# hsinnan75/Dart

Hardware: AMD Instinct MI355X
Metric: M paired-end reads/sec (2x101 bp vs GRCh38-sized index), host to host; records bit-identical to CPU dart (higher is better)
Workload: dtype u64/u8 integer

## Files before the change

### dart_amd/csrc/dg_api.hip

```cpp
#include "../../include/dartgpu.h"
#include "dg_common.h"
#include "dg_fm.h"
#include "dg_seedq.h"
#include "dg_chain.h"
#include "dg_report.h"
#include "dg_pair.h"
#include "dg_reseed.h"
#include "dg_sort.h"
#include "dg_samfmt.h"
#include "dg_bamfmt.h"
#include "dg_bgzf.h"
#include "dg_fastq.h"
#include "dg_sjtab.h"
#include <stdio.h>
#include <stdlib.h>
#include <string.h>
#include <string>
#include <algorithm>
#include <vector>
#include <atomic>
#include <mutex>
#include <chrono>
#include <thread>
#include <condition_variable>
// ... 52 lines not shown
       TOP_ORDER_INFO = 28 , TOP_CLASS_HIST = 32 , TOP_CLASS_FILL = 64  };

struct IndexShared {
    std::mutex mu;
    std::condition_variable cv;
    DIndex ix{};
    std::atomic<uint32_t> gen{1};
    std::thread aids;
    std::atomic<int> aids_state{0};
    char aids_msg[256] = "";
    bool upload_done = false, upload_ok = false;
    void *d_ktab = nullptr, *d_sa_dense = nullptr;
    std::string report, report_out;
    int device = 0;
    uint32_t *d_chr_name_off = nullptr; char *d_chr_names = nullptr; bool chr_names_set = false; uint64_t chr_names_gen = 0; uint32_t chr_name_max = 0;
};

struct dg_ctx {
    int device = 0;
    IndexShared *shared_ix = nullptr; uint32_t ix_gen = 0;
    bool owns_index = true;
    hipStream_t stream = nullptr;
    hipEvent_t ev_dl = nullptr, ev_dl_block = nullptr;
    bool dl_on_copy_stream = false;
    int env_copy_stream = 1;
    hipEvent_t ev_wait = nullptr;
    char err[512] = "";
    DIndex ix{};
    DParams pr{};
    void *d_bwt = nullptr, *d_sa = nullptr, *d_pac = nullptr, *d_lockey = nullptr, *d_locchr = nullptr, *d_chroff = nullptr;
    int n_reads = 0, max_rlen = 0;
    size_t seq_bytes = 0;
    bool enc_ready = false;
    DBuf<unsigned char> seq; DBuf<uint32_t> seq_off; DBuf<uint16_t> rlen; DBuf<uint32_t> enc; DBuf<uint32_t> packed_in, nlist_in;
    DBuf<DHit> hits; DBuf<uint32_t> nhits, nseeds, seed_off, ncand, rep_off, tile_sums, tile_read, slow_units;
    DBuf<SKey> seeds; DBuf<DSeed> work; DBuf<DCand> cands; DBuf<DJob> jobs; DBuf<unsigned long long> job_items, job_pool; DBuf<RsChunkOut> job_outs; DBuf<uint32_t> job_pool_next; DBuf<unsigned long long> items; DBuf<uint32_t> hist, heavy; DBuf<DHeavy> seed_heavy; DBuf<int32_t> seed_heavy_sfail; DBuf<int16_t> chain_picks; DBuf<uint8_t> chain_todo;
    DBuf<dg_read_out> reads_out; DBuf<dg_report_out> reports; DBuf<uint32_t> cigpool, cigfinal;
    DBuf<dg_sj_out> sjpool, sjfinal;
    DBuf<dg_read_c> reads_c; DBuf<dg_report_c> reports_c; DBuf<uint32_t> cig_c;
    DBuf<unsigned char> ws;
    DBuf<unsigned long long> scan_state, scan_trace;
    int wall_khz = 100000;
    uint32_t scan_epoch = 0;
    size_t cap_seeds = 0, cap_rep = 0, cap_work = 0, cap_cig = 0;
    struct SharedCaps { std::atomic<size_t> seeds{0}, rep{0}, work{0}, cig{0}; } *shared_caps = nullptr;
    bool owns_shared_caps = false;
    unsigned long long *d_ctr = nullptr; unsigned int *d_tops = nullptr; int *d_err = nullptr; DSizes *d_sizes = nullptr; unsigned int *d_input_bad = nullptr;
    struct HostTail { DSizes sizes; int err; unsigned int input_bad; unsigned int tops[N_TOPS]; unsigned long long ctr[CTR_STRIDE]; __host__ __device__ uint32_t *sizes_words() { return (uint32_t *)&sizes; } } *h_tail = nullptr;
    bool state_zeroed = false;
    size_t used[3] = {0, 0, 0};
    bool enqueued = false;
    hipEvent_t ev[N_TIMERS + 1]; const char *tname[N_TIMERS]; int n_t = 0; float tms[N_TIMERS];
    uint64_t counters[CTR_N];
    uint64_t reruns_capacity = 0, reruns_scan = 0;
    bool want_compact = true, packed_valid = false;
    DBuf<uint32_t> sam_hdr_off, sam_qual_off, sam_qlen; DBuf<char> sam_hdr, sam_qual, sam_text; DBuf<uint64_t> sam_read_off, sam_tile;
    unsigned long long *d_sam_stat = nullptr, *h_sam_stat = nullptr;
    hipEvent_t ev_sam[2] = {nullptr, nullptr};
    bool batch_done = false, sam_valid = false; size_t sam_bytes = 0;
    DBuf<unsigned char> fq_text; DBuf<uint32_t> fq_lines, fq_tile_cnt, fq_name_at, fq_name_len, fq_loc, fq_hdr_off, fq_qual_off; DBuf<unsigned long long> fq_tile_sum; DBuf<char> fq_hdr, fq_qual;
    FqInfo *d_fq_info = nullptr, *h_fq_info = nullptr;
    hipEvent_t ev_fq[2] = {nullptr, nullptr};
    bool fq_valid = false; size_t fq_hdr_bytes = 0, fq_qual_bytes = 0; float fq_ms = 0.f;
    DBuf<unsigned char> bam_rec, bgzf_in, bgzf_slots, bgzf_out; DBuf<uint32_t> bgzf_size; DBuf<uint64_t> bgzf_off;
    unsigned long long *d_bam_stat = nullptr, *h_bam_stat = nullptr;
    hipEvent_t ev_bam[2] = {nullptr, nullptr}; float bam_ms[2] = {0.f, 0.f};
    bool bam_valid = false; size_t bam_bytes = 0; unsigned char *bam_ptr = nullptr;
    SjSlot *sj_tab = nullptr; size_t sj_slots = 0, sj_distinct = 0;
    DBuf<dg_sj_entry> sj_ovf[2], sj_in, sj_entries; int sj_ovf_cur = 0;
    DBuf<uint64_t> sj_keys[2], sj_line_off, sj_tile; DBuf<int64_t> sj_vals[2]; DBuf<uint32_t> sj_hist, sj_sums; DBuf<char> sj_text;
    unsigned long long *d_sj_stat = nullptr, *h_sj_stat = nullptr;
    hipEvent_t ev_sj[3] = {nullptr, nullptr, nullptr};
    bool sj_batch_counted = false, sj_fin_valid = false; size_t sj_fin_entries = 0, sj_fin_bytes = 0;
    size_t env_bam_first_cap = 0;
    size_t env_sam_first_cap = 0;
    bool want_full = true, full_valid = false;
    int n_cu = 256, runs_of_last_batch = 0, attempt_no = 0;
    int env_seed_waves = 4, env_bail_trips = 0 , env_report_bpc = 8, env_no_fast = 0, env_seed_legacy = 0, env_seed_slots_lg = 0, env_seed_wgs = 0, env_blocking_sync = 0;
    int env_seed_phases = 0, env_seed_wg_waves = 4, env_seed_partial = 32, env_seed_multi = 4;
    bool seed_qf_used = false;
    int env_scan_mask = 7;
    int env_chain_bpc = 8, env_seedh_bpc = 8, env_reseed_pct = 100;
    int env_rs_chunk = RS_CHUNK_DIAGS, env_rs_inline = RS_ENT_INLINE, env_rs_pool = 0;
    int env_scan_budget = 0;
};

static void read_env(dg_ctx *c)
{
    auto geti = [](const char *k, int dflt) { const char *v = getenv(k); return v ? atoi(v) : dflt; };
    c->env_seed_waves = geti("DG_SEED_WAVES", 4); c->env_bail_trips = geti("DG_SEED_BAIL_TRIPS", 0);
    c->env_seed_legacy = geti("DG_SEED_LEGACY", 0); c->env_seed_slots_lg = geti("DG_SEED_SLOTS_LG", 0); c->env_seed_wgs = geti("DG_SEED_WGS", 0); c->env_blocking_sync = geti("DG_BLOCKING_SYNC", 0);
    c->env_report_bpc = geti("DG_REPORT_BPC", 8); c->env_no_fast = geti("DG_NO_FAST_PAIR", 0);
    c->env_scan_budget = geti("DG_SCAN_POLL_BUDGET", 0); c->env_scan_mask = geti("DG_SCAN_POLL_SCANS", 7);
    c->env_seed_phases = geti("DG_SEED_PHASES", 0); c->env_seed_wg_waves = geti("DG_SEED_WG_WAVES", 4); c->env_seed_partial = geti("DG_SEED_PARTIAL_MIN", 32);
    c->env_copy_stream = geti("DG_COPY_STREAM", 1);
    c->env_chain_bpc = std::max(1, geti("DG_CHAIN_BPC", 8)); c->env_seedh_bpc = std::max(1, geti("DG_SEEDH_BPC", 8)); c->env_reseed_pct = std::max(10, geti("DG_RESEED_PCT", 100));
    c->env_rs_chunk = geti("DG_RS_CHUNK", RS_CHUNK_DIAGS); c->env_rs_chunk = std::min(1 << 24, std::max(RS_SUPER, c->env_rs_chunk / RS_SUPER * RS_SUPER));
    c->env_rs_inline = std::min(RS_ENT_INLINE, std::max(0, geti("DG_RS_ENT_MAX", RS_ENT_INLINE))); c->env_rs_pool = std::max(0, geti("DG_RS_POOL_BLOCKS", 0));
    c->env_sam_first_cap = (size_t)std::max(0, geti("DG_SAM_TEXT_FIRST_CAP", 0));
    c->env_bam_first_cap = (size_t)std::max(0, geti("DG_BAM_FIRST_CAP", 0));
    c->env_seed_multi = geti("DG_SEED_MULTI", 4); if (c->env_seed_multi < 0 || c->env_seed_multi > SQF_MULTI_MAX) c->env_seed_multi = SQF_MULTI_MAX;
}

static inline void refresh_index(dg_ctx *c)
{
    IndexShared *sh = c->shared_ix;
    if (sh && c->ix_gen != sh->gen.load(std::memory_order_acquire)) { std::lock_guard<std::mutex> lk(sh->mu); c->ix = sh->ix; c->ix_gen = sh->gen.load(); }
}

static int fail(dg_ctx *c, int code, const char *what, hipError_t e)
{
    snprintf(c ? c->err : g_init_error, 512, "%s: %s", what, e == hipSuccess ? "error" : hipGetErrorString(e));
    return code;
}
#define HIPCHK(call) do { hipError_t _e = (call); if (_e != hipSuccess) return fail(c, DG_ERR_HIP, #call, _e); } while (0)

#define SCAN_TILE 2048
__global__ void __launch_bounds__(256) k_scan_tiles(const uint32_t *in, uint32_t *out, uint32_t *tile_sums, uint32_t n)
{
    __shared__ uint32_t sh[256];
    const uint32_t base = blockIdx.x * SCAN_TILE + threadIdx.x * 8;
    uint32_t v[8], sum = 0;
    for (int i = 0; i < 8; i++) { v[i] = base + i < n ? in[base + i] : 0; sum += v[i]; }
    sh[threadIdx.x] = sum;
    __syncthreads();
    for (int o = 1; o < 256; o <<= 1) {
        uint32_t t = threadIdx.x >= o ? sh[threadIdx.x - o] : 0;
        __syncthreads();
        sh[threadIdx.x] += t;
        __syncthreads();
    }
    uint32_t run = sh[threadIdx.x] - sum;
    for (int i = 0; i < 8; i++) { if (base + i < n) out[base + i] = run; run += v[i]; }
    if (threadIdx.x == 255) tile_sums[blockIdx.x] = sh[255];
}
__global__ void __launch_bounds__(256) k_scan_top(uint32_t *tile_sums, uint32_t n_tiles, uint32_t *total_out, uint32_t *total_copy, uint32_t cap, int *err, int code)
{
    __shared__ uint32_t sh[256];
    __shared__ uint32_t carry;
    if (threadIdx.x == 0) carry = 0;
    __syncthreads();
    for (uint32_t b = 0; b < n_tiles; b += 256) {
        const uint32_t i = b + threadIdx.x;
        const uint32_t v = i < n_tiles ? tile_sums[i] : 0;
        sh[threadIdx.x] = v;
        __syncthreads();
        for (int o = 1; o < 256; o <<= 1) {
            uint32_t t = threadIdx.x >= o ? sh[threadIdx.x - o] : 0;
            __syncthreads();
            sh[threadIdx.x] += t;
            __syncthreads();
        }
        if (i < n_tiles) tile_sums[i] = carry + sh[threadIdx.x] - v;
        __syncthreads();
        if (threadIdx.x == 255) carry += sh[255];
        __syncthreads();
    }
    if (threadIdx.x == 0) {
        *total_out = carry;
        if (total_copy) *total_copy = carry;
        if (err && carry > cap) atomicMax(err, code);
    }
}
__global__ void __launch_bounds__(256) k_scan_add(uint32_t *out, const uint32_t *tile_sums, uint32_t n)
{
    const uint32_t i = blockIdx.x * 256 + threadIdx.x;
    if (i < n) out[i] += tile_sums[i / SCAN_TILE];
}

#define SO_PER 8
__global__ void __launch_bounds__(256)
k_seed_offsets(int n_reads, int paired, const uint32_t *__restrict__ nseeds, uint32_t *__restrict__ seed_off, uint32_t *__restrict__ tile_read, uint32_t n_tile_read,
               uint32_t *__restrict__ heavy_list, unsigned int *n_heavy, uint32_t *total_copy, uint32_t cap, TileScan ts, int *err)
{
    __shared__ unsigned long long s_scan[20];
// ... 631 lines not shown
{
    auto bad = [&](int code, const char *fmt, const char *arg) -> dg_ctx * {
        snprintf(g_init_error, sizeof g_init_error, fmt, arg);
        if (status) *status = code;
        return nullptr;
    };
    if (!f || !p || !f->bwt_path || !f->sa_path || !f->pac_path || f->n_chr <= 0 || !f->chr_off || !f->chr_len || f->l_pac <= 0) return bad(DG_ERR_ARG, "dg_init_files arguments: %s", "invalid");
    struct Fd { int fd = -1; ~Fd() { if (fd >= 0) close(fd); } } fb, fs, fp;
    struct stat st;
    IndexMeta m;
    if ((fb.fd = open(f->bwt_path, O_RDONLY)) < 0 || fstat(fb.fd, &st) != 0 || st.st_size < 40) return bad(DG_ERR_ARG, "cannot read %s", f->bwt_path);
    uint64_t hdr[7];
    if (pread(fb.fd, hdr, 40, 0) != 40) return bad(DG_ERR_ARG, "cannot read %s", f->bwt_path);
    m.primary = hdr[0]; m.L2[0] = 0; for (int i = 1; i < 5; i++) m.L2[i] = hdr[i]; m.seq_len = m.L2[4];
    m.bwt_words = ((uint64_t)st.st_size - 40) / 4;
    if ((fs.fd = open(f->sa_path, O_RDONLY)) < 0 || fstat(fs.fd, &st) != 0 || st.st_size < 56) return bad(DG_ERR_ARG, "cannot read %s", f->sa_path);
    if (pread(fs.fd, hdr, 56, 0) != 56) return bad(DG_ERR_ARG, "cannot read %s", f->sa_path);
    m.sa_intv = (int)hdr[5];
    if (m.sa_intv <= 0 || m.seq_len == 0) return bad(DG_ERR_ARG, "%s: bad header", f->sa_path);
    m.n_sa = (m.seq_len + (uint64_t)m.sa_intv) / (uint64_t)m.sa_intv;
    const uint64_t sa_count = std::min<uint64_t>(m.n_sa - 1, ((uint64_t)st.st_size - 56) / 8);
    if ((fp.fd = open(f->pac_path, O_RDONLY)) < 0 || fstat(fp.fd, &st) != 0) return bad(DG_ERR_ARG, "cannot read %s", f->pac_path);
    const size_t pac_copy = std::min<size_t>((size_t)st.st_size, (size_t)(f->l_pac / 4 + 1));
    m.l_pac = f->l_pac; m.n_chr = f->n_chr; m.chr_off = f->chr_off; m.chr_len = f->chr_len; m.expected_reads = f->expected_reads;
    UpSrc b, s, q;
    b.fd = fb.fd; s.fd = fs.fd; q.fd = fp.fd;
    return init_index(m, b, 40, s, 56, 1, sa_count, q, pac_copy, p, device, flags, status);
}

extern "C" dg_ctx *dg_clone(dg_ctx *parent, int *status)
{
    if (status) *status = DG_ERR_ARG;
    if (!parent) return nullptr;
    hipError_t e;
    if ((e = hipSetDevice(parent->device)) != hipSuccess) { if (status) *status = DG_ERR_HIP; return nullptr; }
    dg_ctx *c = new dg_ctx();
    c->device = parent->device; c->owns_index = false; c->n_cu = parent->n_cu;
    c->shared_ix = parent->shared_ix;
    c->ix = parent->ix; c->ix_gen = parent->ix_gen; c->pr = parent->pr;
    refresh_index(c);
    c->shared_caps = parent->shared_caps;
    if ((e = make_ctx_objects(c)) != hipSuccess) {
        snprintf(g_init_error, sizeof g_init_error, "dg_clone: %s", hipGetErrorString(e)); dg_destroy(c); if (status) *status = DG_ERR_HIP; return nullptr;
    }
    const int live = g_live_ctx[c->device & 63].load();
    if (live + 2 > g_hwq_left && !g_hwq_warned.exchange(true))
        fprintf(stderr, "[libdartgpu] %d contexts on device %d + the copy stream + the caller's stream are more than the %d hardware queues of this process "
                        "(GPU_MAX_HW_QUEUES was %s when the library loaded and %d when its constructor returned): contexts will share queues and wait for each other\n",
                live, c->device, g_hwq_left, g_hwq_found, g_hwq_left);
    if (status) *status = DG_OK;
    return c;
}

static int enqueue_upload(dg_ctx *c, int n_reads, const uint32_t *seq_off, const uint16_t *rlen, const char *seq)
{
    if (!c || n_reads < 0 || (n_reads > 0 && (!seq_off || !rlen || !seq))) return DG_ERR_ARG;
    HIPCHK(hipSetDevice(c->device));
    size_t bytes = 0; int mx = 0;
    for (int i = 0; i < n_reads; i++) {
        const size_t end = (size_t)seq_off[i] + rlen[i];
        bytes = end > bytes ? end : bytes;
        mx = rlen[i] > mx ? rlen[i] : mx;
    }
    if (mx > DG_MAX_RLEN) { snprintf(c->err, 512, "a read is longer than DG_MAX_RLEN (%d)", DG_MAX_RLEN); return DG_ERR_ARG; }
    c->n_reads = n_reads; c->max_rlen = mx; c->seq_bytes = bytes; c->enc_ready = false; c->enqueued = false; c->batch_done = false; c->sj_batch_counted = false; c->sam_valid = false; c->bam_valid = false; c->fq_valid = false;
    HIPCHK(c->seq.ensure(bytes + 64));
    HIPCHK(c->seq_off.ensure((size_t)n_reads + 1)); HIPCHK(c->rlen.ensure((size_t)n_reads + 1));
    if (n_reads) {
        HIPCHK(hipMemcpyAsync(c->seq.p, seq, bytes, hipMemcpyHostToDevice, c->stream));
        HIPCHK(hipMemcpyAsync(c->seq_off.p, seq_off, (size_t)n_reads * 4, hipMemcpyHostToDevice, c->stream));
        HIPCHK(hipMemcpyAsync(c->rlen.p, rlen, (size_t)n_reads * 2, hipMemcpyHostToDevice, c->stream));
    }
    return DG_OK;
}

extern "C" int dg_batch_upload(dg_ctx *c, int n_reads, const uint32_t *seq_off, const uint16_t *rlen, const char *seq)
{
    const int rc = enqueue_upload(c, n_reads, seq_off, rlen, seq);
    if (rc) return rc;
    HIPCHK(hipStreamSynchronize(c->stream));
    return DG_OK;
}

__global__ void __launch_bounds__(256)
k_unpack(const uint32_t *__restrict__ words, uint32_t n_words, int W2, double inv_w2, int rlen_all, const uint16_t *rlen_in, unsigned char *__restrict__ seq,
         uint32_t *__restrict__ seq_off, uint16_t *rlen_out, uint32_t *__restrict__ enc, unsigned int *bad)
{
    const uint32_t t = blockIdx.x * blockDim.x + threadIdx.x;
    if (t >= n_words) return;
    if (t == 0) *bad = 0u;
    uint32_t r = (uint32_t)((double)t * inv_w2);
    if (r * (uint32_t)W2 > t) r--; else if ((r + 1u) * (uint32_t)W2 <= t) r++;
    const int ww = (int)(t - r * (uint32_t)W2);
    const int len = rlen_in ? rlen_in[r] : rlen_all, left = len - 16 * ww;
    const uint32_t w = words[t];
    const uint32_t past = left >= 16 ? 0u : (left <= 0 ? 0xFFFFFFFFu : 0xFFFFFFFFu >> (2 * left));
    enc[(size_t)r * 2 * W2 + ww] = w & ~past;
    enc[(size_t)r * 2 * W2 + W2 + ww] = past;
    if (ww == 0) { seq_off[r] = r * 16u * (uint32_t)W2; if (!rlen_in) rlen_out[r] = (uint16_t)len; }
}
__global__ void __launch_bounds__(256)
k_unpack_n(const uint32_t *__restrict__ nlist, uint32_t n_n, int W2, uint32_t n_bases, unsigned char *__restrict__ seq, uint32_t *__restrict__ enc, unsigned int *bad)
{
    const uint32_t i = blockIdx.x * blockDim.x + threadIdx.x;
    if (i >= n_n) return;
    const uint32_t flat = nlist[i], per = 16u * (uint32_t)W2, r = flat / per, pos = flat - r * per;
    if (flat >= n_bases) { atomicMax(bad, 1u); return; }
    const uint32_t bit = 3u << (30 - 2 * (pos & 15u));
    atomicAnd(&enc[(size_t)r * 2 * W2 + (pos >> 4)], ~bit);
    atomicOr(&enc[(size_t)r * 2 * W2 + W2 + (pos >> 4)], bit);
}

static int enqueue_upload_packed(dg_ctx *c, int n_reads, int rlen_all, const uint16_t *rlen, int words_per_read, const uint32_t *words, const uint32_t *nlist, size_t n_n)
{
    if (!c || n_reads < 0 || words_per_read < 1 || (n_reads > 0 && !words) || (n_n > 0 && !nlist)) return DG_ERR_ARG;
    HIPCHK(hipSetDevice(c->device));
    const int W2 = words_per_read;
    int mx = rlen_all;
    if (rlen) { mx = 0; for (int i = 0; i < n_reads; i++) mx = rlen[i] > mx ? rlen[i] : mx; }
    if (mx > DG_MAX_RLEN || mx > 16 * W2 || (size_t)n_reads * 16 * W2 > 0xFFFFFFF0ull) { snprintf(c->err, 512, "packed batch: read length %d does not fit %d words (or exceeds DG_MAX_RLEN / 2^32 bases)", mx, W2); return DG_ERR_ARG; }
    if (n_reads && (mx + 15) / 16 != W2) { snprintf(c->err, 512, "packed batch: words_per_read must be ceil(longest read / 16) = %d", (mx + 15) / 16); return DG_ERR_ARG; }
    const size_t nw = (size_t)n_reads * W2, bytes = nw * 16;
    c->n_reads = n_reads; c->max_rlen = mx; c->seq_bytes = bytes; c->enqueued = false; c->batch_done = false; c->sj_batch_counted = false; c->sam_valid = false; c->bam_valid = false; c->fq_valid = false;
    HIPCHK(c->seq.ensure(bytes + 64)); HIPCHK(c->seq_off.ensure((size_t)n_reads + 1)); HIPCHK(c->rlen.ensure((size_t)n_reads + 1));
    HIPCHK(c->enc.ensure(2 * nw + 16)); HIPCHK(c->packed_in.ensure(nw + 1)); HIPCHK(c->nlist_in.ensure(n_n + 1));
    c->enc_ready = true;
    if (n_reads == 0) return DG_OK;
    HIPCHK(hipMemcpyAsync(c->packed_in.p, words, nw * 4, hipMemcpyHostToDevice, c->stream));
    if (rlen) HIPCHK(hipMemcpyAsync(c->rlen.p, rlen, (size_t)n_reads * 2, hipMemcpyHostToDevice, c->stream));
    if (n_n) HIPCHK(hipMemcpyAsync(c->nlist_in.p, nlist, n_n * 4, hipMemcpyHostToDevice, c->stream));
    k_unpack<<<(unsigned)((nw + 255) / 256), 256, 0, c->stream>>>(c->packed_in.p, (uint32_t)nw, W2, 1.0 / (double)W2, rlen_all, rlen ? c->rlen.p : nullptr, c->seq.p, c->seq_off.p, c->rlen.p, c->enc.p, c->d_input_bad);
    if (n_n) {
        k_unpack_n<<<(unsigned)((n_n + 255) / 256), 256, 0, c->stream>>>(c->nlist_in.p, (uint32_t)n_n, W2, (uint32_t)(nw * 16), c->seq.p, c->enc.p, c->d_input_bad);
        HIPCHK(hipMemcpyAsync(&c->h_tail->input_bad, c->d_input_bad, 4, hipMemcpyDeviceToHost, c->stream));
    } else c->h_tail->input_bad = 0;
    HIPCHK(hipGetLastError());
    return DG_OK;
}

extern "C" int dg_batch_upload_packed(dg_ctx *c, int n_reads, int rlen_all, const uint16_t *rlen, int words_per_read, const uint32_t *words, const uint32_t *nlist, size_t n_n)
{
    const int rc = enqueue_upload_packed(c, n_reads, rlen_all, rlen, words_per_read, words, nlist, n_n);
    if (rc) return rc;
    HIPCHK(hipStreamSynchronize(c->stream));
    return DG_OK;
}

extern "C" int dg_fastq_tile(void) { return FQ_TILE; }

extern "C" int dg_batch_upload_fastq(dg_ctx *c, const dg_fastq_text *in, int *n_reads_out)
{
    if (!c) return DG_ERR_ARG;
    if (n_reads_out) *n_reads_out = 0;
    c->n_reads = 0; c->max_rlen = 0; c->seq_bytes = 0; c->enc_ready = false; c->enqueued = false; c->batch_done = false; c->sj_batch_counted = false; c->sam_valid = false; c->bam_valid = false; c->fq_valid = false;
    c->fq_hdr_bytes = c->fq_qual_bytes = 0; c->fq_ms = 0.f;
    if (!in) { snprintf(c->err, 512, "dg_batch_upload_fastq: the input is NULL"); return DG_ERR_ARG; }
    const size_t n1 = in->text1 ? in->n1 : 0, n2 = in->text2 ? in->n2 : 0;
    const bool two = in->text2 != nullptr && in->n2 > 0;
    if ((in->n1 && !in->text1) || in->max_reads < 0) { snprintf(c->err, 512, "dg_batch_upload_fastq: text1 is NULL or max_reads is negative"); return DG_ERR_ARG; }
    if (n1 >= 0xFFFFFF00ull || n2 >= 0xFFFFFF00ull) { snprintf(c->err, 512, "dg_batch_upload_fastq: a text must be smaller than 2^32 - 256 bytes"); return DG_ERR_ARG; }
    if (n1 == 0 && !two) { c->fq_valid = true; return DG_OK; }
    HIPCHK(hipSetDevice(c->device));
    if (!c->d_fq_info) {
        HIPCHK(hipMalloc((void **)&c->d_fq_info, sizeof(FqInfo)));
        HIPCHK(hipHostMalloc((void **)&c->h_fq_info, sizeof(FqInfo), hipHostMallocDefault));
        for (hipEvent_t &e : c->ev_fq) HIPCHK(hipEventCreate(&e));
    }
    const size_t max_reads = (size_t)in->max_reads;
    const size_t rec_cap[2] = { two ? (max_reads + 1) / 2 : max_reads, two ? max_reads / 2 : 0 };
    const size_t nb[2] = { n1, n2 };
    size_t line_cap[2], tiles[2];
    for (int f = 0; f < 2; f++) { line_cap[f] = std::min(4 * rec_cap[f] + 1, nb[f] + 1); tiles[f] = (nb[f] + FQ_TILE - 1) / FQ_TILE; }
    const size_t off2 = (n1 + 16 + 255) & ~(size_t)255, text_bytes = n1 + n2;
    const size_t tile_stride = std::max(tiles[0], tiles[1]);
    const size_t reads_bound = std::min(max_reads, (n1 + 4) / 4 + (n2 + 4) / 4);
    const size_t len_tiles = std::max<size_t>(1, (reads_bound + FQ_THREADS - 1) / FQ_THREADS);
    HIPCHK(c->fq_text.ensure(off2 + n2 + 32)); HIPCHK(c->fq_lines.ensure(line_cap[0] + line_cap[1] + 2)); HIPCHK(c->fq_tile_cnt.ensure(2 * tile_stride + 1));
    HIPCHK(c->fq_name_at.ensure(reads_bound + 1)); HIPCHK(c->fq_name_len.ensure(reads_bound + 1)); HIPCHK(c->fq_loc.ensure(3 * (reads_bound + 1))); HIPCHK(c->fq_tile_sum.ensure(3 * len_tiles));
    HIPCHK(c->fq_hdr_off.ensure(reads_bound + 1)); HIPCHK(c->fq_qual_off.ensure(reads_bound + 1)); HIPCHK(c->fq_hdr.ensure(text_bytes + 1)); HIPCHK(c->fq_qual.ensure(text_bytes + 1));
    HIPCHK(c->seq.ensure(text_bytes + 64)); HIPCHK(c->seq_off.ensure(reads_bound + 1)); HIPCHK(c->rlen.ensure(reads_bound + 1));
    if (n1) HIPCHK(hipMemcpyAsync(c->fq_text.p, in->text1, n1, hipMemcpyHostToDevice, c->stream));
    if (n2) HIPCHK(hipMemcpyAsync(c->fq_text.p + off2, in->text2, n2, hipMemcpyHostToDevice, c->stream));
    FqText x;
    x.t[0] = c->fq_text.p; x.t[1] = c->fq_text.p + off2; x.n[0] = (uint32_t)n1; x.n[1] = (uint32_t)n2;
    x.line_start[0] = c->fq_lines.p; x.line_start[1] = c->fq_lines.p + line_cap[0] + 1; x.line_cap[0] = (uint32_t)line_cap[0]; x.line_cap[1] = (uint32_t)line_cap[1];
    x.two = two ? 1 : 0;
    const uint32_t stride = (uint32_t)(reads_bound + 1);
    const dim3 text_grid((unsigned)std::max<size_t>(1, tile_stride), two ? 2u : 1u);
    HIPCHK(hipEventRecord(c->ev_fq[0], c->stream));
    k_fq_count<<<text_grid, FQ_THREADS, 0, c->stream>>>(x, c->fq_tile_cnt.p, (uint32_t)tile_stride);
    k_fq_top<<<1, FQ_THREADS, 0, c->stream>>>(x, c->fq_tile_cnt.p, (uint32_t)tile_stride, (uint32_t)max_reads, c->d_fq_info);
    k_fq_lines<<<text_grid, FQ_THREADS, 0, c->stream>>>(x, c->fq_tile_cnt.p, (uint32_t)tile_stride, c->d_fq_info);
    k_fq_len<<<(unsigned)len_tiles, FQ_THREADS, 0, c->stream>>>(x, c->d_fq_info, c->rlen.p, c->fq_name_at.p, c->fq_name_len.p, c->fq_loc.p, stride, c->fq_tile_sum.p, (uint32_t)len_tiles);
    k_fq_top3<<<1, FQ_THREADS, 0, c->stream>>>(c->fq_tile_sum.p, (uint32_t)len_tiles, c->d_fq_info);
    if (reads_bound)
        k_fq_write<<<(unsigned)reads_bound, 64, 0, c->stream>>>(x, c->d_fq_info, in->rc_odd_reads ? 1 : 0, c->rlen.p, c->fq_name_at.p, c->fq_name_len.p, c->fq_loc.p, stride, c->fq_tile_sum.p,
                                                                 (uint32_t)len_tiles, c->seq_off.p, c->seq.p, c->fq_hdr_off.p, c->fq_hdr.p, c->fq_qual_off.p, c->fq_qual.p);
    HIPCHK(hipGetLastError());
    HIPCHK(hipEventRecord(c->ev_fq[1], c->stream));
    HIPCHK(hipMemcpyAsync(c->h_fq_info, c->d_fq_info, sizeof(FqInfo), hipMemcpyDeviceToHost, c->stream));
    HIPCHK(wait_stream(c));
    (void)hipEventElapsedTime(&c->fq_ms, c->ev_fq[0], c->ev_fq[1]);
    const FqInfo &fi = *c->h_fq_info;
    if (n_reads_out) *n_reads_out = (int)std::min<uint32_t>(fi.n_reads, 0x7FFFFFFFu);
    switch (fi.status) {
    case FQ_OK: break;
    case FQ_E_COUNT:
        snprintf(c->err, 512, "dg_batch_upload_fastq: text1 holds %u records and text2 %u: they must be equal, or text1 one more", (fi.n_lines[0] + 3) / 4, (fi.n_lines[1] + 3) / 4);
        return DG_ERR_ARG;
    case FQ_E_CAPACITY:
        snprintf(c->err, 512, "dg_batch_upload_fastq: the texts hold %u reads, max_reads is %d", fi.n_reads, in->max_reads);
        return DG_ERR_CAPACITY;
    case FQ_E_EMPTY:
        snprintf(c->err, 512, "dg_batch_upload_fastq: read %u is a record without bases", fi.bad_read);
// ... 85 lines not shown
    int lg = 0;
    while ((1 << lg) < W / 2) lg++;
    if (!c->enc_ready) k_encode<<<(unsigned)((((size_t)n << lg) + 255) / 256), 256, 0, c->stream>>>(c->seq.p, c->seq_off.p, c->rlen.p, n, W, lg, c->enc.p);
    if (after_encode) { e = hipEventRecord(after_encode, c->stream); if (e != hipSuccess) return e; }
    if ((e = c->seed_heavy.ensure((size_t)n + 16)) != hipSuccess) return e;
    unsigned blocks = (unsigned)c->n_cu * (unsigned)c->env_seed_waves;
    if ((size_t)blocks * 64 > (size_t)n) blocks = (unsigned)((n + 63) / 64);
    const bool use_qf = !c->env_seed_legacy && !c->env_seed_phases && W <= 62 && c->pr.max_dup <= 30000;
    const int bail_trips = c->env_bail_trips > 0 ? c->env_bail_trips : (use_qf ? 64 : 128);
    unsigned int *tops = c->d_tops;
    c->seed_qf_used = false;
    if (use_qf) {
        int lg = c->env_seed_slots_lg >= 6 && c->env_seed_slots_lg <= 11 ? c->env_seed_slots_lg : 9;
        int nw = c->env_seed_wg_waves >= 1 && c->env_seed_wg_waves <= 8 ? c->env_seed_wg_waves : 4;
        while (lg > 6 && sqf_lds_bytes(lg, W, nw) > (size_t)156 * 1024) lg--;
        if (c->env_seed_slots_lg == 0) while (lg > 6 && sqf_lds_bytes(lg, W, nw) > (size_t)80 * 1024) lg--;
        const size_t lds = sqf_lds_bytes(lg, W, nw);
        if ((e = raise_dynamic_lds((const void *)k_seed_qf, 0, c->device, lds)) != hipSuccess) return e;
        unsigned per_cu = (unsigned)(((size_t)160 * 1024) / lds);
        if (per_cu * (unsigned)nw > 16u) per_cu = 16u / (unsigned)nw;
        if (per_cu > 2u) per_cu = 2u;
        if (per_cu < 1u) per_cu = 1u;
        if (c->env_seed_wgs > 0) per_cu = (unsigned)c->env_seed_wgs;
        unsigned wgs = (unsigned)c->n_cu * per_cu;
        const unsigned need = (unsigned)(((size_t)n + ((size_t)1 << lg) - 1) >> lg);
        if (wgs > need) wgs = need;
        c->seed_qf_used = true;
        k_seed_qf<<<wgs, nw * 64, lds, c->stream>>>(c->ix, c->pr, c->enc.p, c->rlen.p, n, W, H, lg, c->hits.p, c->nhits.p, c->nseeds.p, tops + TOP_SEED_NEXT,
                                                    c->seed_heavy.p, tops + TOP_SEED_HEAVY, c->d_ctr, bail_trips, c->env_seed_partial, c->env_seed_multi, c->d_err, bail_trips);
    } else
    if (!c->env_seed_legacy && W <= 62) {
        int lg = c->env_seed_slots_lg >= 6 && c->env_seed_slots_lg <= 10 ? c->env_seed_slots_lg : 9;
        while (lg > 6 && sq_lds_bytes(lg, W) > (size_t)80 * 1024) lg--;
        const size_t lds = sq_lds_bytes(lg, W);
        if ((e = raise_dynamic_lds((const void *)k_seed_q, 1, c->device, lds)) != hipSuccess) return e;
        unsigned per_cu = (unsigned)(((size_t)160 * 1024) / lds);
        if (per_cu > 4u) per_cu = 4u;
        if (c->env_seed_wgs > 0) per_cu = (unsigned)c->env_seed_wgs;
        unsigned wgs = (unsigned)c->n_cu * per_cu;
        const unsigned need = (unsigned)(((size_t)n + ((size_t)1 << lg) - 1) >> lg);
        if (wgs > need) wgs = need;
        k_seed_q<<<wgs, SQ_THREADS, lds, c->stream>>>(c->ix, c->pr, c->enc.p, c->rlen.p, n, W, H, lg, c->hits.p, c->nhits.p, c->nseeds.p, tops + TOP_SEED_NEXT,
                                                      c->seed_heavy.p, tops + TOP_SEED_HEAVY, c->d_ctr, bail_trips, c->d_err);
    } else
    if (W <= 78) k_seed<true><<<blocks, 64, ((size_t)2 * W * 64 + 64) * 4, c->stream>>>(c->ix, c->pr, c->enc.p, c->rlen.p, n, W, H, c->hits.p, c->nhits.p, c->nseeds.p, tops + TOP_SEED_NEXT, c->seed_heavy.p, tops + TOP_SEED_HEAVY, c->d_ctr, bail_trips);
    else k_seed<false><<<blocks, 64, 0, c->stream>>>(c->ix, c->pr, c->enc.p, c->rlen.p, n, W, H, c->hits.p, c->nhits.p, c->nseeds.p, tops + TOP_SEED_NEXT, c->seed_heavy.p, tops + TOP_SEED_HEAVY, c->d_ctr, bail_trips);
    if ((e = c->seed_heavy_sfail.ensure((size_t)n + 16)) != hipSuccess) return e;
    k_seed_heavy_walk<<<(unsigned)c->n_cu * 8u, 64, 0, c->stream>>>(c->ix, c->pr, c->enc.p, c->rlen.p, W, c->seed_heavy.p, tops + TOP_SEED_HEAVY, c->seed_heavy_sfail.p, c->d_ctr);
    k_seed_heavy<<<(unsigned)c->n_cu * (unsigned)c->env_seedh_bpc, 64, (size_t)W * 4 + 16, c->stream>>>(c->ix, c->pr, c->enc.p, c->rlen.p, W, H, c->hits.p, c->nhits.p, c->nseeds.p, c->seed_heavy.p, tops + TOP_SEED_HEAVY, c->seed_heavy_sfail.p, c->d_ctr);
    return hipGetLastError();
}

static TileScan make_tile_scan(dg_ctx *c, size_t first_tile, unsigned int *ticket, int which )
{
    TileScan ts;
    ts.w = c->scan_state.p + SCAN_WORDS * first_tile; ts.ticket = ticket; ts.epoch = c->scan_epoch;
    ts.budget = (c->env_scan_budget > 0 && c->attempt_no == 0 && (c->env_scan_mask & which)) ? (uint32_t)c->env_scan_budget : 0u;
    ts.dbg = c->d_sizes->scan_dbg;
    ts.ticks = (unsigned long long)c->wall_khz * 2000ull;
    ts.trace = c->scan_trace.p ? c->scan_trace.p + SCAN_TRACE_WORDS * first_tile : nullptr;
    return ts;
}

#define TICK(name) do { if (c->n_t < N_TIMERS) { c->tname[c->n_t] = name; HIPCHK(hipEventRecord(c->ev[c->n_t + 1], c->stream)); c->n_t++; } } while (0)

static int enqueue_seeding(dg_ctx *c, int n, int H, bool timed, bool paired_units)
{
    HIPCHK(c->hits.ensure((size_t)n * H)); HIPCHK(c->nhits.ensure(n)); HIPCHK(c->nseeds.ensure(n)); HIPCHK(c->seed_off.ensure((size_t)n + 1));
    if (c->shared_caps) caps_adopt(c->cap_seeds, c->shared_caps->seeds);
    if (c->cap_seeds < (size_t)n * 3 + 1024) c->cap_seeds = (size_t)n * 3 + 1024;
    HIPCHK(c->seeds.ensure(c->cap_seeds + 1)); HIPCHK(c->cands.ensure(c->cap_seeds + 1)); HIPCHK(c->tile_read.ensure(c->cap_seeds / 64 + 16));
    if (timed) c->tname[c->n_t] = "k_encode";
    HIPCHK(launch_seed(c, n, H, timed ? c->ev[c->n_t + 1] : nullptr));
    if (timed) { c->n_t++; TICK("k_seed"); }
    {
        const int paired = (paired_units && (n % 2 == 0)) ? 1 : 0;
        HIPCHK(c->heavy.ensure((size_t)n + 16));
        const TileScan ts_seed = make_tile_scan(c, 0, c->d_tops + TOP_TICKET_SEED, 1);
        k_seed_offsets<<<(unsigned)((n + 256 * SO_PER - 1) / (256 * SO_PER)), 256, 0, c->stream>>>(n, paired, c->nseeds.p, c->seed_off.p, c->tile_read.p, (uint32_t)c->tile_read.cap,
                                                                                                 c->heavy.p, c->d_tops + TOP_HEAVY_UNITS, &c->d_sizes->total_seeds, (uint32_t)c->cap_seeds, ts_seed, c->d_err);
        HIPCHK(hipGetLastError());
    }
    if (timed) TICK("seed_offsets");
    k_locate<<<(unsigned)((c->cap_seeds + 255) / 256), 256, 0, c->stream>>>(c->ix, n, H, c->hits.p, c->tile_read.p, c->seed_off.p, c->seeds.p, c->d_ctr, c->d_err);
    HIPCHK(hipGetLastError());
    if (timed) TICK("k_locate");
    return DG_OK;
}

__global__ void __launch_bounds__(256)
k_batch_begin(unsigned long long *ctr, unsigned int *tops, int *err, DSizes *sizes)
{
    for (int i = threadIdx.x; i < CTR_STRIPES * CTR_STRIDE; i += 256) ctr[i] = 0ull;
    if (threadIdx.x < N_TOPS) tops[threadIdx.x] = 0u;
    if (threadIdx.x < (int)(sizeof(DSizes) / 4)) ((uint32_t *)sizes)[threadIdx.x] = 0u;
    if (threadIdx.x == 0) *err = 0;
}

static size_t scan_tiles_seed(int n_reads) { return (size_t)(n_reads + 256 * SO_PER - 1) / (256 * SO_PER) + 1; }
static size_t scan_tiles_pair(int n_units) { return (size_t)(n_units + PU_THREADS - 1) / PU_THREADS + 1; }

__global__ void __launch_bounds__(256)
k_batch_end(DSizes *__restrict__ sizes, int *__restrict__ err, unsigned int *__restrict__ tops, unsigned long long *__restrict__ ctr, dg_ctx::HostTail *out)
{
    const int t = threadIdx.x;
    if (t < (int)(sizeof(DSizes) / 4)) { out->sizes_words()[t] = ((const uint32_t *)sizes)[t]; ((uint32_t *)sizes)[t] = 0u; }
    if (t < N_TOPS) { out->tops[t] = tops[t]; tops[t] = 0u; }
    if (t == 0) { out->err = *err; *err = 0; }
    if (t < CTR_STRIDE) {
        const bool is_max = t == CTR_MAXTRIPS || t == CTR_WTRIPS_MAX;
        unsigned long long v = 0;
        for (int s_ = 0; s_ < CTR_STRIPES; s_++) { const unsigned long long x = ctr[s_ * CTR_STRIDE + t]; ctr[s_ * CTR_STRIDE + t] = 0ull; v = is_max ? (x > v ? x : v) : v + x; }
        out->ctr[t] = v;
    }
}

static int zero_batch_state(dg_ctx *c, int n_reads, int n_units)
{
    if (!c->state_zeroed) {
        k_batch_begin<<<1, 256, 0, c->stream>>>(c->d_ctr, c->d_tops, c->d_err, c->d_sizes);
        HIPCHK(hipGetLastError());
    }
    c->state_zeroed = false;
    const size_t tiles2 = (size_t)(2 * n_units + 255) / 256 + 1;
    const size_t words = SCAN_WORDS * (scan_tiles_seed(n_reads) + scan_tiles_pair(n_units) + tiles2);
    if (words > c->scan_state.cap) {
        HIPCHK(c->scan_state.ensure(words));
        HIPCHK(hipMemsetAsync(c->scan_state.p, 0, c->scan_state.cap * 8, c->stream));
        static_assert(SCAN_TRACE_WORDS == SCAN_WORDS, "the trace array is sized like the state array");
        HIPCHK(c->scan_trace.ensure(c->scan_state.cap));
        HIPCHK(hipMemsetAsync(c->scan_trace.p, 0, c->scan_trace.cap * 8, c->stream));
    }
    c->scan_epoch = (c->scan_epoch + 1u) & 0x3FFFFFFFu;
    if (c->scan_epoch == 0) c->scan_epoch = 1;
    return DG_OK;
}


static int enqueue_run(dg_ctx *c)
{
    const int n = c->n_reads;
    const int paired = (c->pr.paired && (n % 2 == 0)) ? 1 : 0;
    const int n_units = paired ? n / 2 : n;
    refresh_index(c);
    c->n_t = 0;
    const int H = c->max_rlen / 16 + 1;
    const uint32_t nb = (uint32_t)((n + 255) / 256);
    { const int zr = zero_batch_state(c, n, n_units); if (zr) return zr; }
    HIPCHK(hipEventRecord(c->ev[0], c->stream));
    { const int rc = enqueue_seeding(c, n, H, true, c->pr.paired != 0); if (rc) return rc; }

    if (c->shared_caps) { caps_adopt(c->cap_rep, c->shared_caps->rep); caps_adopt(c->cap_cig, c->shared_caps->cig); caps_adopt(c->cap_work, c->shared_caps->work); }
    if (c->cap_rep < (size_t)n + (size_t)n / 4 + 1024) c->cap_rep = (size_t)n + (size_t)n / 4 + 1024;
    if (c->cap_cig < 3 * c->cap_rep) c->cap_cig = 3 * c->cap_rep;
    if (c->cap_work < (size_t)n * 8 + 65536) c->cap_work = (size_t)n * 8 + 65536;
    const size_t cigcap = (size_t)n * 48 + c->cap_rep * (16 + CIG_SLOT) + 4096, sjcap = (size_t)n * 4 + 1024;
    HIPCHK(c->ncand.ensure(n)); HIPCHK(c->rep_off.ensure((size_t)n + 1)); HIPCHK(c->reads_out.ensure(n));
    HIPCHK(c->heavy.ensure((size_t)n_units + 16)); HIPCHK(c->slow_units.ensure((size_t)n_units + 16));
    HIPCHK(c->reports.ensure(c->cap_rep + 1)); HIPCHK(c->work.ensure(c->cap_work + 16)); HIPCHK(c->jobs.ensure(c->cap_seeds + 16));
    const uint32_t rs_out_cap = (uint32_t)std::max<size_t>(16384, (size_t)n / 8), rs_list_cap = (uint32_t)std::min<size_t>(c->jobs.cap + rs_out_cap, 0xFFFFFFF0u);
    HIPCHK(c->job_outs.ensure(rs_out_cap)); HIPCHK(c->job_items.ensure(3 * (size_t)rs_list_cap + 16));
    const uint32_t rs_pool_cap = (uint32_t)std::max<size_t>(16384, (size_t)n / 32);
    HIPCHK(c->job_pool.ensure((size_t)rs_pool_cap * 64)); HIPCHK(c->job_pool_next.ensure(rs_pool_cap));
    HIPCHK(c->cigpool.ensure(cigcap)); HIPCHK(c->cigfinal.ensure(c->cap_cig + 16)); HIPCHK(c->sjpool.ensure(sjcap)); HIPCHK(c->sjfinal.ensure(sjcap));
    HIPCHK(c->items.ensure(c->cap_seeds + 16));
    unsigned int *tops = c->d_tops;

// ... 1283 lines not shown
```

### dart_amd/csrc/dg_fm.h

```cpp
#pragma once
#include "dg_common.h"

struct OccBlock { uint4 q0, q1, q2, q3; };

__device__ __forceinline__ OccBlock d_load_block(const DIndex &ix, uint64_t blk)
{
    const uint4 *p = ix.bwt + (blk << 2);
    OccBlock b;
    b.q0 = p[0]; b.q1 = p[1]; b.q2 = p[2]; b.q3 = p[3];
    return b;
}

__device__ __forceinline__ uint64_t d_sel4(uint64_t a0, uint64_t a1, uint64_t a2, uint64_t a3, int i)
{
    uint64_t lo = (i & 1) ? a1 : a0, hi = (i & 1) ? a3 : a2;
    return (i & 2) ? hi : lo;
}
__device__ __forceinline__ uint64_t d_L2(const DIndex &ix, int i)
{
    return i == 4 ? ix.L2[4] : d_sel4(ix.L2[0], ix.L2[1], ix.L2[2], ix.L2[3], i);
}

__device__ __forceinline__ void d_plane_counts(const uint4 H, const uint4 Lo, uint32_t hmask, uint32_t o, uint32_t &P, uint32_t &Q)
{
// ... 630 lines not shown
                if (acgt && direct && s.mode == 1 && s.x2 == 1) { s.mode = 3; s.lk = s.x0; s.lsteps = 0; }
                while (__ballot(acgt && s.mode != 0)) {
                    t.aux = T_NONE; ta.pa = ta.pb = ta.p16 = nullptr; ta.p8 = nullptr;
                    const int sel = __popcll(__ballot(acgt && s.mode == 1)) >= __popcll(__ballot(acgt && s.mode == 2)) ? 1 : 2;
                    if (acgt && (s.mode == 3 || s.mode == sel)) d_trip_issue(ix, rm, len, direct, s, c, ta, t);
                    d_trip_load(ta, t);
                    if (t.aux != T_NONE) d_trip_finish(ix, pr, rb, rm, len, s, c, t);
                    if (acgt && direct && s.mode == 1 && s.x2 == 1) { s.mode = 3; s.lk = s.x0; s.lsteps = 0; }
                }
            }
            const int nlim = (pos + 64 < end_pos ? pos + 64 : end_pos) - pos;
            const unsigned long long in_round = nlim >= 64 ? ~0ull : ((1ull << nlim) - 1ull);
            const unsigned long long hitm = __ballot(acgt && s.hit_len > 0) & in_round;
            unsigned long long vis = 0;
            int cur = 0;
            while (cur < nlim) {
                const unsigned long long m = hitm >> cur;
                if (!m) { vis |= in_round & ~((1ull << cur) - 1ull); cur = nlim; break; }
                const int j = cur + (__ffsll((long long)m) - 1);
                vis |= (j >= 63 ? ~0ull : ((1ull << (j + 1)) - 1ull)) & ~((1ull << cur) - 1ull);
                cur = j + __shfl(s.hit_len, j, 64);
            }
            const bool seen = (vis >> lane) & 1ull;
            if (seen && doomed) { c.steps += (unsigned long long)(len - st - 1); c.blocks += 2ull * (unsigned long long)(len - st - 1); }
            if (seen && acgt) { c.steps += s.ref_steps; c.blocks += s.ref_blocks; }
            const unsigned long long vh = vis & hitm;
            if ((vh >> lane) & 1ull) {
                const int at = nh + __popcll(vh & ((1ull << lane) - 1ull));
                if (at < H) {
                    DHit h; h.rPos = (uint16_t)s.start; h.len = (uint16_t)s.hit_len;
                    if (s.located) { h.x0 = (uint64_t)s.tpos; h.freq = 1u | 0x80000000u; c.lf_ref += s.lsteps + (uint32_t)(s.lk >> 40); }
                    else { h.x0 = s.x0; h.freq = (uint32_t)s.x2; }
                    hits[(size_t)r * H + at] = h;
                }
            }
            uint32_t fr = ((vh >> lane) & 1ull) ? (uint32_t)s.x2 : 0u;
            for (int o = 32; o > 0; o >>= 1) fr += (uint32_t)__shfl_xor((int)fr, o, 64);
            nh += __popcll(vh); ns += fr;
            cur += pos;
            pos = cur;
        }
        if (lane == 0) { nhits[r] = (uint32_t)nh; nseeds[r] = ns; }
    }
    d_wave_add(ctr + CTR_STEPS, c.steps);
    d_wave_add(ctr + CTR_BLOCKS, c.blocks);
    d_wave_add(ctr + CTR_STEPS_ACT, c.steps_act);
    d_wave_add(ctr + CTR_BLOCKS_ACT, c.blocks_act);
    d_wave_add(ctr + CTR_KTAB, c.ktab);
    d_wave_add(ctr + CTR_LF, c.lf_ref);
    d_wave_add(ctr + CTR_LF_ACT, c.lf_act);
    d_wave_add(ctr + CTR_DIRECT, c.n_direct);
    d_wave_resident(ctr, CTR_WT_SEEDH, t_wave0);
}

__global__ void __launch_bounds__(256)
k_build_sa_dense(const DIndex ix, int intv, uint64_t n_entries, uint64_t *__restrict__ dense)
{
    const uint64_t smask = (uint64_t)ix.sa_intv - 1, dmask = (uint64_t)intv - 1;
    const uint64_t n_sampled = (ix.seq_len + (uint64_t)ix.sa_intv) / (uint64_t)ix.sa_intv;
    int dsh = 0;
    while ((1 << dsh) < intv) dsh++;
    for (uint64_t q = (uint64_t)blockIdx.x * blockDim.x + threadIdx.x; q < n_sampled; q += (uint64_t)gridDim.x * blockDim.x) {
        const uint64_t r0 = q * (uint64_t)ix.sa_intv;
        if ((r0 >> dsh) < n_entries) dense[r0 >> dsh] = ((ix.sa[q] + 1) & 0xFFFFFFFFFFull);
        uint64_t k = d_lf(ix, r0), T = 1;
        while (k & smask) { k = d_lf(ix, k); T++; }
        const uint64_t base = ix.sa[k / (uint64_t)ix.sa_intv];
        k = d_lf(ix, r0);
        for (uint64_t t = 1; t < T; t++) {
            const uint64_t steps = T - t;
            if (!(k & dmask) && (k >> dsh) < n_entries) dense[k >> dsh] = ((steps + base + 1) & 0xFFFFFFFFFFull) | (steps << 40);
            k = d_lf(ix, k);
        }
    }
}


__global__ void __launch_bounds__(256)
k_locate(const DIndex ix, int n_reads, int H, const DHit *__restrict__ hits, const uint32_t *__restrict__ tile_read,
         const uint32_t *__restrict__ seed_off, SKey *__restrict__ seeds, unsigned long long *ctr, const int *__restrict__ abort_p)
{
    if (*abort_p >= DG_ABORT) return;
    const uint32_t total = seed_off[n_reads];
    const int lane = threadIdx.x & 63;
    const uint32_t tile = blockIdx.x * (blockDim.x >> 6) + (threadIdx.x >> 6);
    const uint32_t u = (tile << 6) + (uint32_t)lane;
    unsigned long long lf = 0, lf_act = 0, nsa = 0;
    if ((tile << 6) < total) {
        int r0 = (int)tile_read[tile];
        const uint32_t u_last = (tile << 6) + 63 < total ? (tile << 6) + 63 : total - 1;
        int r = -1;
        uint32_t first = 0;
        while (true) {
            const int rr = r0 + lane;
            const uint32_t nxt = rr + 1 <= n_reads ? seed_off[rr + 1] : 0xFFFFFFFFu;
            int lo = 0;
#pragma unroll
            for (int step = 32; step > 0; step >>= 1) {
                const uint32_t v = __shfl(nxt, lo + step - 1, 64);
                if (v <= u) lo += step;
            }
            if (__shfl(nxt, lo, 64) <= u) lo++;
            const uint32_t win_end = __shfl(nxt, 63, 64);
            if (r < 0 && u < total && lo < 64) { r = r0 + lo; first = seed_off[r]; }
            if (win_end > u_last) break;
            r0 += 64;
        }
        if (u < total) {
            uint32_t w = u - first;
            const DHit *h = hits + (size_t)r * H;
            uint32_t fr = h->freq;
            while (w >= (fr & 0x7FFFFFFFu)) { w -= fr & 0x7FFFFFFFu; h++; fr = h->freq; }
            uint64_t k = h->x0 + w;
            uint64_t steps = 0, pos;
            if (fr & 0x80000000u) pos = h->x0;
            else if (ix.sa_dense) {
                const uint64_t mask = (uint64_t)ix.sa_dense_intv - 1;
                while (k & mask) { k = d_lf(ix, k); steps++; }
                const uint64_t e = ix.sa_dense[k >> ix.sa_dense_shift];
                pos = steps + (e & 0xFFFFFFFFFFull) - 1;
                lf += steps + (e >> 40); lf_act += steps;
            } else {
                const uint64_t mask = (uint64_t)ix.sa_intv - 1;
                while (k & mask) { k = d_lf(ix, k); steps++; }
                pos = steps + ix.sa[k / (uint64_t)ix.sa_intv];
                lf += steps; lf_act += steps;
            }
            nsa++;
            seeds[u] = sk_make((int64_t)pos, (int)h->rPos, (int)h->len);
        }
    }
    d_wave_add(ctr + CTR_LF, lf);
    d_wave_add(ctr + CTR_LF_ACT, lf_act);
    d_wave_add(ctr + CTR_SA, nsa);
}
```

Baseline: 1174.

## Make locate and unpack kernels persistent grid-stride with coalesced unpack layout

k_locate becomes a persistent grid-stride kernel whose grid is capped at n_cu times a configurable blocks-per-CU value, and it loads each DHit once as a struct. k_unpack is rewritten as a templated grid-stride kernel that walks 64-read blocks per wave with byte-offset arithmetic, replacing the per-thread double-precision division, and it precomputes the tail mask when all reads share one length. The aim is to cut launch and tail overhead and index arithmetic, at the cost of fewer waves in flight to hide latency in the memory-bound LF walks.

```diff
diff --git a/dart_amd/csrc/dg_api.hip b/dart_amd/csrc/dg_api.hip
--- a/dart_amd/csrc/dg_api.hip
+++ b/dart_amd/csrc/dg_api.hip
@@ -158,6 +158,7 @@
     int env_scan_mask = 7;
     int env_chain_bpc = 8, env_seedh_bpc = 8, env_reseed_pct = 100;
     int env_rs_chunk = RS_CHUNK_DIAGS, env_rs_inline = RS_ENT_INLINE, env_rs_pool = 0;
+    int env_locate_bpc = 8;
     int env_scan_budget = 0;
 };
 
@@ -166,7 +167,7 @@
     auto geti = [](const char *k, int dflt) { const char *v = getenv(k); return v ? atoi(v) : dflt; };
     c->env_seed_waves = geti("DG_SEED_WAVES", 4); c->env_bail_trips = geti("DG_SEED_BAIL_TRIPS", 0);
     c->env_seed_legacy = geti("DG_SEED_LEGACY", 0); c->env_seed_slots_lg = geti("DG_SEED_SLOTS_LG", 0); c->env_seed_wgs = geti("DG_SEED_WGS", 0); c->env_blocking_sync = geti("DG_BLOCKING_SYNC", 0);
-    c->env_report_bpc = geti("DG_REPORT_BPC", 8); c->env_no_fast = geti("DG_NO_FAST_PAIR", 0);
+    c->env_report_bpc = geti("DG_REPORT_BPC", 8); c->env_locate_bpc = std::min(32, std::max(0, geti("DG_LOCATE_BPC", 8))); c->env_no_fast = geti("DG_NO_FAST_PAIR", 0);
     c->env_scan_budget = geti("DG_SCAN_POLL_BUDGET", 0); c->env_scan_mask = geti("DG_SCAN_POLL_SCANS", 7);
     c->env_seed_phases = geti("DG_SEED_PHASES", 0); c->env_seed_wg_waves = geti("DG_SEED_WG_WAVES", 4); c->env_seed_partial = geti("DG_SEED_PARTIAL_MIN", 32);
     c->env_copy_stream = geti("DG_COPY_STREAM", 1);
@@ -964,22 +965,40 @@
     return DG_OK;
 }
 
+template <bool PER_READ>
 __global__ void __launch_bounds__(256)
-k_unpack(const uint32_t *__restrict__ words, uint32_t n_words, int W2, double inv_w2, int rlen_all, const uint16_t *rlen_in, unsigned char *__restrict__ seq,
+k_unpack(const uint32_t *__restrict__ words, uint32_t n_reads, uint32_t W2, uint32_t q64, uint32_t m64, int rlen_all, uint32_t tail, const uint16_t *rlen_in,
          uint32_t *__restrict__ seq_off, uint16_t *rlen_out, uint32_t *__restrict__ enc, unsigned int *bad)
 {
-    const uint32_t t = blockIdx.x * blockDim.x + threadIdx.x;
-    if (t >= n_words) return;
-    if (t == 0) *bad = 0u;
-    uint32_t r = (uint32_t)((double)t * inv_w2);
-    if (r * (uint32_t)W2 > t) r--; else if ((r + 1u) * (uint32_t)W2 <= t) r++;
-    const int ww = (int)(t - r * (uint32_t)W2);
-    const int len = rlen_in ? rlen_in[r] : rlen_all, left = len - 16 * ww;
-    const uint32_t w = words[t];
-    const uint32_t past = left >= 16 ? 0u : (left <= 0 ? 0xFFFFFFFFu : 0xFFFFFFFFu >> (2 * left));
-    enc[(size_t)r * 2 * W2 + ww] = w & ~past;
-    enc[(size_t)r * 2 * W2 + W2 + ww] = past;
-    if (ww == 0) { seq_off[r] = r * 16u * (uint32_t)W2; if (!rlen_in) rlen_out[r] = (uint16_t)len; }
+    const uint32_t gt = blockIdx.x * 256u + threadIdx.x, n_threads = gridDim.x * 256u;
+    if (gt == 0) *bad = 0u;
+    for (uint32_t r = gt; r < n_reads; r += n_threads) { seq_off[r] = r * 16u * W2; if (!PER_READ) rlen_out[r] = (uint16_t)rlen_all; }
+    const uint32_t lane = threadIdx.x & 63u, wave = (uint32_t)__builtin_amdgcn_readfirstlane((int)(gt >> 6)), n_waves = n_threads >> 6;
+    const uint32_t n_blocks = (n_reads + 63u) >> 6, n_words = n_reads * W2, block_words = 64u * W2;
+    const uint32_t n_full = n_reads >> 6, step_in = n_waves * block_words * 4u;
+    const char *const in = (const char *)words;
+    char *const lo_plane = (char *)enc, *const hi_plane = (char *)(enc + W2);
+    auto word = [&](uint32_t b, uint32_t q, uint32_t m, uint32_t off_in, uint32_t off_e, uint32_t past) {
+        const uint32_t w = *(const uint32_t *)(in + off_in);
+        if (PER_READ) {
+            const int left = (int)rlen_in[b * 64u + q] - 16 * (int)m;
+            past = left >= 16 ? 0u : (left <= 0 ? 0xFFFFFFFFu : 0xFFFFFFFFu >> (2 * left));
+        }
+        *(uint32_t *)(lo_plane + off_e) = w & ~past;
+        *(uint32_t *)(hi_plane + off_e) = past;
+    };
+    uint32_t q = lane / W2, m = lane - q * W2;
+    for (uint32_t j = 0; j < W2; j++) {
+        const uint32_t past = m == W2 - 1u ? tail : 0u;
+        const uint32_t t = wave * block_words + j * 64u + lane;
+        uint32_t off_in = t * 4u, off_e = (t + (wave * 64u + q) * W2) * 4u;
+        uint32_t b = wave;
+#pragma unroll 2
+        for (; b < n_full; b += n_waves, off_in += step_in, off_e += 2u * step_in) word(b, q, m, off_in, off_e, past);
+        if (b == n_full && n_full < n_blocks && off_in < n_words * 4u) word(b, q, m, off_in, off_e, past);
+        q += q64; m += m64;
+        if (m >= W2) { m -= W2; q++; }
+    }
 }
 __global__ void __launch_bounds__(256)
 k_unpack_n(const uint32_t *__restrict__ nlist, uint32_t n_n, int W2, uint32_t n_bases, unsigned char *__restrict__ seq, uint32_t *__restrict__ enc, unsigned int *bad)
@@ -1011,7 +1030,15 @@
     HIPCHK(hipMemcpyAsync(c->packed_in.p, words, nw * 4, hipMemcpyHostToDevice, c->stream));
     if (rlen) HIPCHK(hipMemcpyAsync(c->rlen.p, rlen, (size_t)n_reads * 2, hipMemcpyHostToDevice, c->stream));
     if (n_n) HIPCHK(hipMemcpyAsync(c->nlist_in.p, nlist, n_n * 4, hipMemcpyHostToDevice, c->stream));
-    k_unpack<<<(unsigned)((nw + 255) / 256), 256, 0, c->stream>>>(c->packed_in.p, (uint32_t)nw, W2, 1.0 / (double)W2, rlen_all, rlen ? c->rlen.p : nullptr, c->seq.p, c->seq_off.p, c->rlen.p, c->enc.p, c->d_input_bad);
+    {
+        const unsigned n_blocks = ((unsigned)n_reads + 63u) / 64u, wgs = std::min((unsigned)c->n_cu * 4u, (n_blocks + 15u) / 16u);
+        const uint32_t uW2 = (uint32_t)W2, q64 = 64u / uW2, m64 = 64u % uW2;
+        if (rlen) k_unpack<true><<<wgs, 256, 0, c->stream>>>(c->packed_in.p, (uint32_t)n_reads, uW2, q64, m64, 0, 0u, c->rlen.p, c->seq_off.p, c->rlen.p, c->enc.p, c->d_input_bad);
+        else {
+            const int left = rlen_all - 16 * (W2 - 1);
+            k_unpack<false><<<wgs, 256, 0, c->stream>>>(c->packed_in.p, (uint32_t)n_reads, uW2, q64, m64, rlen_all, left >= 16 ? 0u : 0xFFFFFFFFu >> (2 * left), nullptr, c->seq_off.p, c->rlen.p, c->enc.p, c->d_input_bad);
+        }
+    }
     if (n_n) {
         k_unpack_n<<<(unsigned)((n_n + 255) / 256), 256, 0, c->stream>>>(c->nlist_in.p, (uint32_t)n_n, W2, (uint32_t)(nw * 16), c->seq.p, c->enc.p, c->d_input_bad);
         HIPCHK(hipMemcpyAsync(&c->h_tail->input_bad, c->d_input_bad, 4, hipMemcpyDeviceToHost, c->stream));
@@ -1263,7 +1290,8 @@
         HIPCHK(hipGetLastError());
     }
     if (timed) TICK("seed_offsets");
-    k_locate<<<(unsigned)((c->cap_seeds + 255) / 256), 256, 0, c->stream>>>(c->ix, n, H, c->hits.p, c->tile_read.p, c->seed_off.p, c->seeds.p, c->d_ctr, c->d_err);
+    const size_t locate_wgs = std::min((c->cap_seeds + 255) / 256, std::max((size_t)1, (size_t)c->n_cu * (size_t)c->env_locate_bpc));
+    k_locate<<<(unsigned)locate_wgs, 256, 0, c->stream>>>(c->ix, n, H, c->hits.p, c->tile_read.p, c->seed_off.p, c->seeds.p, c->d_ctr, c->d_err);
     HIPCHK(hipGetLastError());
     if (timed) TICK("k_locate");
     return DG_OK;
diff --git a/dart_amd/csrc/dg_fm.h b/dart_amd/csrc/dg_fm.h
--- a/dart_amd/csrc/dg_fm.h
+++ b/dart_amd/csrc/dg_fm.h
@@ -736,11 +736,13 @@
 {
     if (*abort_p >= DG_ABORT) return;
     const uint32_t total = seed_off[n_reads];
+    const uint32_t n_tiles = (total >> 6) + ((total & 63u) ? 1u : 0u);
     const int lane = threadIdx.x & 63;
-    const uint32_t tile = blockIdx.x * (blockDim.x >> 6) + (threadIdx.x >> 6);
-    const uint32_t u = (tile << 6) + (uint32_t)lane;
-    unsigned long long lf = 0, lf_act = 0, nsa = 0;
-    if ((tile << 6) < total) {
+    const uint32_t n_waves = gridDim.x * (blockDim.x >> 6);
+    unsigned long long lf = 0, lf_act = 0;
+    uint32_t nsa = 0;
+    for (uint32_t tile = (uint32_t)__builtin_amdgcn_readfirstlane((int)(blockIdx.x * (blockDim.x >> 6) + (threadIdx.x >> 6))); tile < n_tiles; tile += n_waves) {
+        const uint32_t u = (tile << 6) + (uint32_t)lane;
         int r0 = (int)tile_read[tile];
         const uint32_t u_last = (tile << 6) + 63 < total ? (tile << 6) + 63 : total - 1;
         int r = -1;
@@ -763,28 +765,32 @@
         if (u < total) {
             uint32_t w = u - first;
             const DHit *h = hits + (size_t)r * H;
-            uint32_t fr = h->freq;
-            while (w >= (fr & 0x7FFFFFFFu)) { w -= fr & 0x7FFFFFFFu; h++; fr = h->freq; }
-            uint64_t k = h->x0 + w;
-            uint64_t steps = 0, pos;
-            if (fr & 0x80000000u) pos = h->x0;
-            else if (ix.sa_dense) {
-                const uint64_t mask = (uint64_t)ix.sa_dense_intv - 1;
-                while (k & mask) { k = d_lf(ix, k); steps++; }
-                const uint64_t e = ix.sa_dense[k >> ix.sa_dense_shift];
-                pos = steps + (e & 0xFFFFFFFFFFull) - 1;
-                lf += steps + (e >> 40); lf_act += steps;
-            } else {
-                const uint64_t mask = (uint64_t)ix.sa_intv - 1;
-                while (k & mask) { k = d_lf(ix, k); steps++; }
-                pos = steps + ix.sa[k / (uint64_t)ix.sa_intv];
-                lf += steps; lf_act += steps;
+            DHit hv = *h;
+            while (w >= (hv.freq & 0x7FFFFFFFu)) { w -= hv.freq & 0x7FFFFFFFu; h++; hv = *h; }
+            uint64_t pos = hv.x0;
+            const bool walk = !(hv.freq & 0x80000000u);
+            if (__ballot(walk)) {
+                if (walk) {
+                    uint64_t k = hv.x0 + w, steps = 0;
+                    if (ix.sa_dense) {
+                        const uint64_t mask = (uint64_t)ix.sa_dense_intv - 1;
+                        while (k & mask) { k = d_lf(ix, k); steps++; }
+                        const uint64_t e = ix.sa_dense[k >> ix.sa_dense_shift];
+                        pos = steps + (e & 0xFFFFFFFFFFull) - 1;
+                        lf += steps + (e >> 40); lf_act += steps;
+                    } else {
+                        const uint64_t mask = (uint64_t)ix.sa_intv - 1;
+                        while (k & mask) { k = d_lf(ix, k); steps++; }
+                        pos = steps + ix.sa[k / (uint64_t)ix.sa_intv];
+                        lf += steps; lf_act += steps;
+                    }
+                }
             }
             nsa++;
-            seeds[u] = sk_make((int64_t)pos, (int)h->rPos, (int)h->len);
+            seeds[u] = sk_make((int64_t)pos, (int)hv.rPos, (int)hv.len);
         }
     }
     d_wave_add(ctr + CTR_LF, lf);
     d_wave_add(ctr + CTR_LF_ACT, lf_act);
-    d_wave_add(ctr + CTR_SA, nsa);
-}
+    d_wave_add(ctr + CTR_SA, (unsigned long long)nsa);
+}
```

After: 1169. Within noise of the previous version (-0.5%).
